# nurturenature/jepsen-tigerbeetle

Hardware: NVIDIA H100
Metric: configs explored/sec (time-to-verdict alongside) on 10k-op/32-client bank history (higher is better)
Workload: dtype int64

## Files before the change

### jepsen_tigerbeetle_b200/csrc/jtb_abi.cu

```cuda
#include <algorithm>
#include <chrono>
#include <cstdio>
#include <cstdlib>
#include <cstring>
#include <mutex>
#include <string>
#include <thread>
#include <type_traits>
#include <vector>

#include "jtb_wgl.cuh"
#include "jtb_level.cuh"
#include "jtb_scout.cuh"
#include "jtb_scans.cuh"
#include "jtb_table_bench.cuh"
#include "jtb_partition.cuh"
#include "jtb_monotonic.cuh"
#include "jtb_counter_bounds.cuh"
#include "jtb_transfer_lookups.cuh"
#include "jtb_read_explanations.cuh"
#include "jtb_read_gaps.cuh"
#include "jtb_transfer_placement.cuh"

using namespace jtb;
// ... 44 lines not shown
            return -1;                                                                       \
        }                                                                                    \
    } while (0)

int ensure(jtb_ctx* ctx, DevBuf& b, size_t bytes) {
    if (bytes <= b.cap) return 0;
    if (b.p) CK(cudaFree(b.p));
    b.p = nullptr;
    b.cap = 0;
    size_t want = std::max<size_t>(bytes, 256);
    CK(cudaMalloc(&b.p, want));
    b.cap = want;
    return 0;
}

template <typename T>
int upload(jtb_ctx* ctx, DevBuf& b, const std::vector<T>& v) {
    ctx->stats[12] += v.size() * sizeof(T);
    if (ensure(ctx, b, v.size() * sizeof(T) + 64)) return -1;
    if (!v.empty()) CK(cudaMemcpyAsync(b.p, v.data(), v.size() * sizeof(T), cudaMemcpyHostToDevice, ctx->stream));
    return 0;
}

template <typename F>
int dispatch_model_kw(jtb_ctx* ctx, int kind, int kw, F&& f) {
    using std::integral_constant;
    if (kind == JTB_MODEL_SET) return f(integral_constant<int, JTB_MODEL_SET>(), integral_constant<int, 2>());
    auto by_kw = [&](auto model) -> int {
        switch (kw) {
        case 2: return f(model, integral_constant<int, 2>());
        case 4: return f(model, integral_constant<int, 4>());
        case 8: return f(model, integral_constant<int, 8>());
        }
        ctx->err = "unsupported key width";
        return -1;
    };
    return kind == JTB_MODEL_BANK ? by_kw(integral_constant<int, JTB_MODEL_BANK>())
                                  : by_kw(integral_constant<int, JTB_MODEL_CAS_REGISTER>());
}

template <int MODEL, int KW>
int launch_wgl(jtb_ctx* ctx, const WglParams& p, int neg_ok, int grid, size_t smem) {
    auto k = p.eager_reads ? wgl_search_kernel<MODEL, KW, JTB_CTAS_EAGER, true> : wgl_search_kernel<MODEL, KW, JTB_CTAS_EXACT, false>;
    CK(cudaFuncSetAttribute(k, cudaFuncAttributeMaxDynamicSharedMemorySize, (int)smem));
    k<<<grid, WGL_THREADS, smem, ctx->stream>>>(p, neg_ok);
    CK(cudaGetLastError());
    return 0;
}

template <int MODEL, int KW>
int launch_level(jtb_ctx* ctx, const LvParams& p, int neg_ok, bool eager, int* grid_out) {
    constexpr int EW = KW + (MODEL == JTB_MODEL_BANK ? 4 : 0);
    const bool beam = p.beam_w != 0;
    const size_t smem = (beam ? sizeof(LvScratch<KW, EW, MODEL == JTB_MODEL_BANK, true>)
                              : sizeof(LvScratch<KW, EW, MODEL == JTB_MODEL_BANK, false>)) * LV_WARPS;
    const bool nk = !(MODEL == JTB_MODEL_BANK && !neg_ok);
    const void* k;
#define JTB_LVK(E, N, B) (const void*)level_search_kernel<MODEL, KW, E, (MODEL == JTB_MODEL_BANK ? N : true), B>
    if (beam) k = eager ? (nk ? JTB_LVK(true, true, true) : JTB_LVK(true, false, true)) : (nk ? JTB_LVK(false, true, true) : JTB_LVK(false, false, true));
    else k = eager ? (nk ? JTB_LVK(true, true, false) : JTB_LVK(true, false, false)) : (nk ? JTB_LVK(false, true, false) : JTB_LVK(false, false, false));
#undef JTB_LVK
    CK(cudaFuncSetAttribute(k, cudaFuncAttributeMaxDynamicSharedMemorySize, (int)smem));
    int per_sm = 0;
    CK(cudaOccupancyMaxActiveBlocksPerMultiprocessor(&per_sm, k, LV_THREADS, smem));
    if (per_sm < 1) { ctx->err = "level engine: the kernel does not fit on an SM"; return -1; }
    per_sm = std::min(per_sm, JTB_LV_CTAS);
    const int grid = ctx->opts.search_ctas ? std::min<int>((int)ctx->opts.search_ctas, ctx->n_sms * per_sm) : ctx->n_sms * per_sm;
    if (grid > 1024) { ctx->err = "level engine: more CTAs than barrier release words"; return -1; }
    *grid_out = grid;
    LvParams pp = p;
    void* args[] = {&pp};
    CK(cudaLaunchCooperativeKernel(k, dim3(grid), dim3(LV_THREADS), args, smem, ctx->stream));
    return 0;
}

int search_level(jtb_ctx* ctx, const jtb_model* m, const Prepared& P, int n_shards, const std::vector<int>& searchable,
                 const std::vector<uint64_t>& init_entries, Ctrl& hc, double& kernel_s, uint64_t& configs, uint64_t& probes,
                 uint32_t beam_w = 0) {
    const int KW = P.key_words;
    const bool bank = m->kind == JTB_MODEL_BANK;
    const int EW = KW + (bank ? 4 : 0);
    const bool eager = !(ctx->opts.flags & JTB_OPT_NO_EAGER_READS);
    size_t free_b = 0, total_b = 0;
    CK(cudaMemGetInfo(&free_b, &total_b));
    const size_t reserve = (size_t)4 << 30;
    const size_t avail = ctx->table.cap + ctx->lv_buf[0].cap + ctx->lv_buf[1].cap + (free_b > reserve ? free_b - reserve : 0);
    size_t table_bytes = ctx->opts.table_bytes ? ctx->opts.table_bytes
                         : (getenv("JTB_LV_TABLE_MB") ? (size_t)atoll(getenv("JTB_LV_TABLE_MB")) << 20 : (size_t)1 << 30);
    table_bytes = std::min(table_bytes, avail / 3);
    size_t buf_bytes = getenv("JTB_LV_BUF_MB") ? (size_t)atoll(getenv("JTB_LV_BUF_MB")) << 20 : (size_t)512 << 20;
    buf_bytes = std::max<size_t>(std::min(buf_bytes, avail / 3), init_entries.size() * 8 + 4096);
    auto slots_of = [&](size_t bytes) { uint64_t s = 1; while (s * 2 * KW * 8 <= bytes) s <<= 1; return s; };
    uint64_t table_slots = slots_of(std::max(table_bytes, ctx->table.cap));
    auto ensure_table = [&](uint64_t slots) -> int {
        const void* before = ctx->table.p;
        if (ensure(ctx, ctx->table, slots * KW * 8)) return -1;
        if (ctx->table.p != before) ctx->table_dirty = ~(size_t)0;
        return 0;
    };
    if (ensure_table(table_slots)) return -1;
    if (ensure(ctx, ctx->lv_buf[0], std::max(buf_bytes, ctx->lv_buf[0].cap)) || ensure(ctx, ctx->lv_buf[1], std::max(buf_bytes, ctx->lv_buf[1].cap)) ||
        ensure(ctx, ctx->lv_ctrl, sizeof(LvCtrl)))
        return -1;
    uint64_t buf_cap = std::min(ctx->lv_buf[0].cap, ctx->lv_buf[1].cap) / ((size_t)EW * 8);
    if (beam_w) {
        if (ensure(ctx, ctx->lv_aux[0], buf_cap * 4 + 64) || ensure(ctx, ctx->lv_aux[1], buf_cap * 4 + 64) ||
            ensure(ctx, ctx->lv_beam, sizeof(LvBeam)))
            return -1;
        std::vector<LvBeam> hb(1);
        std::memset(hb.data(), 0, sizeof(LvBeam));
        for (int k = 0; k < 3; ++k)
            for (int s = 0; s < LV_BEAM_SHARDS; ++s) { hb[0].min_crashed[k][s] = 0x7fffffff; hb[0].max_rank[k][s] = -1; }
        for (int s : searchable) { hb[0].min_crashed[0][s] = 0; hb[0].max_rank[0][s] = (int)P.rank_base[s]; }
        CK(cudaMemcpyAsync(ctx->lv_beam.p, hb.data(), sizeof(LvBeam), cudaMemcpyHostToDevice, ctx->stream));
        CK(cudaMemsetAsync(ctx->lv_aux[0].p, 0, init_entries.size() / EW * 4 + 64, ctx->stream));
        CK(cudaStreamSynchronize(ctx->stream));
    }
    CK(cudaMemsetAsync(ctx->table.p, 0, std::min(ctx->table_dirty, (size_t)table_slots * KW * 8), ctx->stream));
    ctx->table_dirty = 0;
    LvCtrl lc;
    std::memset(&lc, 0, sizeof lc);
    lc.n_undecided = (int)searchable.size();
    CK(cudaMemcpyAsync(ctx->lv_ctrl.p, &lc, sizeof lc, cudaMemcpyHostToDevice, ctx->stream));
    CK(cudaMemcpyAsync(ctx->lv_buf[0].p, init_entries.data(), init_entries.size() * 8, cudaMemcpyHostToDevice, ctx->stream));
    LvParams p{};
    p.rows = (const int32_t*)ctx->rows.p;
    p.classes = (const ClassRec*)ctx->classes.p;
    p.cls_inv_pos = (const int32_t*)ctx->cls_inv.p;
    p.ctrl = (LvCtrl*)ctx->lv_ctrl.p;
    p.shard_found = (int*)ctx->found.p;
    p.shard_max_rank = (int*)ctx->maxrank.p;
    p.row_words = P.row_words;
    p.sum_off = P.sum_off;
    p.n_shards = n_shards;
    p.max_configs = ctx->opts.max_configs;
    p.time_budget_ns = (unsigned long long)ctx->opts.time_budget_ms * 1000000ull;
    p.narrow_max = getenv("JTB_LV_NARROW") ? (uint32_t)atoi(getenv("JTB_LV_NARROW")) : (uint32_t)(LV_WARPS * 8);
    p.slots_per_config = getenv("JTB_LV_SPC") ? (uint32_t)std::max(2, atoi(getenv("JTB_LV_SPC"))) : 16u;
    p.min_slots = 1ull << 16;
    std::memset(&p.init, 0, sizeof p.init);
    p.init.n_in = searchable.size();
    p.init.epoch = 1;
    p.init.s_in = 0; p.init.s_out = 1; p.init.s_spare = 2;
    p.init.contig = 1;
    p.init.beam_thr = -1;
    p.init.beam_frac = 1024;
    p.beam_w = beam_w;
    p.aux[0] = (uint32_t*)ctx->lv_aux[0].p;
    p.aux[1] = (uint32_t*)ctx->lv_aux[1].p;
    p.beam = (LvBeam*)ctx->lv_beam.p;
    p.init.win = 0;
    CK(cudaEventRecord(ctx->ev0, ctx->stream));
    int attempts = 0, grid = 0;
    unsigned long long max_window = 0, max_width = 0, narrow_levels = 0, max_probe = 0;
    const double t_begin = now_s();
    for (;;) {
        ++attempts;
        p.table = (uint64_t*)ctx->table.p;
        p.table_slots = table_slots;
        p.min_slots = std::min<uint64_t>(p.min_slots, table_slots);
        p.buf[0] = (uint64_t*)ctx->lv_buf[0].p;
        p.buf[1] = (uint64_t*)ctx->lv_buf[1].p;
        p.buf_cap = buf_cap;
        p.seg_cap = buf_cap / LV_NSEG;
        p.init.zeroed = table_slots;
        p.init.win = lv_window(p, p.init.n_in, 0);
        if (ctx->opts.time_budget_ms) {
            const double left = ctx->opts.time_budget_ms * 1e-3 - (now_s() - t_begin);
            p.time_budget_ns = (unsigned long long)(std::max(left, 1e-3) * 1e9);
        }
        const int neg_ok = bank ? m->negative_balances_ok : 0;
        if (int rc = dispatch_model_kw(ctx, m->kind, KW, [&](auto M, auto K) { return launch_level<M(), K()>(ctx, p, neg_ok, eager, &grid); }))
            return rc;
        CK(cudaMemcpyAsync(&lc, ctx->lv_ctrl.p, sizeof lc, cudaMemcpyDeviceToHost, ctx->stream));
        CK(cudaStreamSynchronize(ctx->stream));
        if (lc.abort) { ctx->err = "level engine: a grid barrier timed out (internal error)"; return -1; }
#ifdef JTB_LV_PROF
        if (beam_w && getenv("JTB_BEAM_TRACE")) {
            for (int i = 0; i < 2048 && (i == 0 || lc.trace[i][1]); ++i)
                if (i < 40 || i % 25 == 0)
                    fprintf(stderr, "[beam W=%u] attempt %d level %d n_out %d thr %d frac %d min_c %d max_r %d\n", beam_w, i, lc.trace[i][0],
                            lc.trace[i][1], lc.trace[i][2], lc.trace[i][3], lc.trace[i][4], lc.trace[i][5]);
        }
        {
            const double wide = (double)std::max<unsigned long long>(lc.prof[9], 1), att = (double)std::max<unsigned long long>(lc.prof[8], 1);
            fprintf(stderr, "[lv prof] attempts %llu (wide %llu)  per attempt, cycles: phase1 %.0f phase2 %.0f flush %.0f | per wide level: "
                    "attempt %.0f barrier %.0f collect %.0f\n", lc.prof[8], lc.prof[9], lc.prof[0] / att, lc.prof[1] / att, lc.prof[2] / att,
                    lc.prof[3] / wide, lc.prof[4] / wide, lc.prof[5] / wide);
            unsigned long long bmin = ~0ull, bmax = 0, bsum = 0, wmin = ~0ull, wmax = 0, wsum = 0;
            for (int i = 0; i < grid; ++i) {
                bmin = std::min(bmin, lc.prof_cta[i][0]); bmax = std::max(bmax, lc.prof_cta[i][0]); bsum += lc.prof_cta[i][0];
                wmin = std::min(wmin, lc.prof_cta[i][1]); wmax = std::max(wmax, lc.prof_cta[i][1]); wsum += lc.prof_cta[i][1];
            }
            fprintf(stderr, "[lv prof] per CTA over the launch, Mcycles: busy min %.1f avg %.1f max %.1f | barrier wait min %.1f avg %.1f max %.1f\n",
                    bmin * 1e-6, bsum * 1e-6 / grid, bmax * 1e-6, wmin * 1e-6, wsum * 1e-6 / grid, wmax * 1e-6);
        }
#endif
        probes += lc.probes;
        max_window = std::max(max_window, lc.max_window);
        max_width = std::max(max_width, lc.max_width);
        max_probe = std::max(max_probe, lc.max_probe_len);
        narrow_levels += lc.narrow_levels;
        ctx->table_dirty = std::max(ctx->table_dirty, (size_t)std::max<uint64_t>(lc.max_window, p.min_slots) * KW * 8);
        if (!(lc.fin.stop == 2 && lc.fin.cause == JTB_CAUSE_TABLE_FULL)) break;
        if (beam_w) break;
        CK(cudaMemGetInfo(&free_b, &total_b));
        const size_t have = ctx->table.cap + ctx->lv_buf[0].cap + ctx->lv_buf[1].cap;
        const size_t room = have + (free_b > reserve ? free_b - reserve : 0);
        const size_t new_table = std::min<size_t>((size_t)table_slots * KW * 8 * 4, (size_t)64 << 30);
        const size_t new_buf = std::min(ctx->lv_buf[0].cap, ctx->lv_buf[1].cap) * 4;
        if (new_table + 2 * new_buf + ctx->lv_buf[lc.fin.in_idx].cap > room) break;
        const int ii = lc.fin.in_idx;
        if (ctx->lv_buf[ii ^ 1].p) { CK(cudaFree(ctx->lv_buf[ii ^ 1].p)); ctx->lv_buf[ii ^ 1] = DevBuf(); }
        if (ctx->table.p) { CK(cudaFree(ctx->table.p)); ctx->table = DevBuf(); }
        DevBuf grown;
        if (ensure(ctx, grown, new_buf)) return -1;
        if (lc.fin.contig) {
            CK(cudaMemcpyAsync(grown.p, ctx->lv_buf[ii].p, (size_t)lc.fin.n_in * EW * 8, cudaMemcpyDeviceToDevice, ctx->stream));
        } else {
            size_t off = 0;
            const size_t seg_cap = buf_cap / LV_NSEG;
            for (int sg = 0; sg < LV_NSEG; ++sg) {
                const size_t n = (size_t)lc.seg[lc.fin.s_in][sg].n;
                if (!n) continue;
                CK(cudaMemcpyAsync((char*)grown.p + off * EW * 8, (const char*)ctx->lv_buf[ii].p + (size_t)sg * seg_cap * EW * 8,
                                   n * EW * 8, cudaMemcpyDeviceToDevice, ctx->stream));
                off += n;
            }
            if (off != lc.fin.n_in) { ctx->err = "level engine: segment counts do not add up"; return -1; }
        }
        CK(cudaStreamSynchronize(ctx->stream));
        CK(cudaFree(ctx->lv_buf[ii].p));
        ctx->lv_buf[ii] = grown;
        if (ensure(ctx, ctx->lv_buf[ii ^ 1], new_buf)) return -1;
        table_slots = slots_of(new_table);
        if (ensure_table(table_slots)) return -1;
        CK(cudaMemsetAsync(ctx->table.p, 0, (size_t)table_slots * KW * 8, ctx->stream));
        ctx->table_dirty = 0;
        buf_cap = new_buf / ((size_t)EW * 8);
        LvState r = lc.fin;
        r.stop = 0; r.cause = 0; r.boost = 0; r.attempt = 0; r.epoch = 1;
        r.s_in = 0; r.s_out = 1; r.s_spare = 2; r.contig = 1;
        p.init = r;
        const int undecided = lc.n_undecided;
        std::memset(&lc, 0, sizeof lc);
        lc.n_undecided = undecided;
        CK(cudaMemcpyAsync(ctx->lv_ctrl.p, &lc, sizeof lc, cudaMemcpyHostToDevice, ctx->stream));
    }
    CK(cudaEventRecord(ctx->ev1, ctx->stream));
    CK(cudaStreamSynchronize(ctx->stream));
    float ms = 0;
    CK(cudaEventElapsedTime(&ms, ctx->ev0, ctx->ev1));
    kernel_s = ms * 1e-3;
    configs = lc.fin.total;
    std::memset(&hc, 0, sizeof hc);
    hc.stop = lc.fin.stop;
    hc.cause = lc.fin.cause;
    hc.configs = lc.fin.total;
    hc.probes = probes;
    hc.n_undecided = lc.n_undecided;
    unsigned long long* st = ctx->stats;
    st[0] = configs; st[1] = probes; st[2] = lc.fin.level + 1; st[3] = max_width; st[4] = narrow_levels; st[5] = 0;
    st[6] = max_probe; st[7] = max_window; st[8] = (unsigned long long)grid; st[9] = buf_cap;
    st[10] = (unsigned long long)attempts; st[11] = (unsigned long long)(ms * 1e3);
    st[12] += init_entries.size() * 8 + sizeof(LvCtrl) + (size_t)n_shards * 4;
    st[13] = (unsigned long long)attempts * sizeof(LvCtrl) + (size_t)n_shards * 8;
    st[14] = (unsigned long long)attempts;
    st[19] = 1;
    return 0;
}

struct ScoutGuard {
    jtb_ctx* ctx;
    bool active = false;
    explicit ScoutGuard(jtb_ctx* c) : ctx(c) {}
    int stop() {
        if (!active) return 0;
        active = false;
        static const unsigned long long one = 1;
        cudaError_t e = cudaMemcpyAsync((unsigned long long*)ctx->sc_ctl.p + 1, &one, 8, cudaMemcpyHostToDevice, ctx->stream);
        if (e == cudaSuccess) e = cudaStreamSynchronize(ctx->scout_stream);
        if (e != cudaSuccess) { ctx->err = std::string("stopping the scouts: ") + cudaGetErrorString(e); return -1; }
        return 0;
    }
    ~ScoutGuard() { stop(); }
};

template <typename K>
int preload(jtb_ctx* ctx, K kernel) {
    cudaFuncAttributes a;
    CK(cudaFuncGetAttributes(&a, kernel));
    return 0;
}

template <int MODEL, int KW>
// ... 800 lines not shown
```

### jepsen_tigerbeetle_b200/csrc/jtb_expand.h

```cpp
#pragma once
#include <cstdint>

#include "jtb_prep.h"

#if defined(__CUDACC__)
#define JTB_HD __host__ __device__ __forceinline__
#else
#define JTB_HD inline
#endif

namespace jtb {

constexpr uint64_t XKEY_VALID = 1ull << 63;
constexpr uint32_t XRANK_MASK = 0x1fffffffu;

struct I4 {
    int32_t x, y, z, w;
};

JTB_HD I4 ld_i4(const int32_t* p) {
#if defined(__CUDA_ARCH__)
    const int4 v = __ldg(reinterpret_cast<const int4*>(p));
    return I4{v.x, v.y, v.z, v.w};
#else
// ... 187 lines not shown
        }
#pragma unroll
        for (int i = 0; i < KW; ++i) ch.w[i] = w[i];
        int cgj = gj;
        if (t == rslot) advance(T, ch.w[1], cgj);
        else ch.w[1] |= 1ull << t;
        ch.w[0] = XKEY_VALID | ((uint64_t)(uint32_t)cgj << 32) | (REG ? (uint64_t)(uint32_t)creg : 0ull);
        ch.cgj = cgj;
        ch.done = cgj >= gj_end;
        return true;
    }

    JTB_HD void load_transfer(int t, Child<KW>& ch) const {
        const I4 op = ld_i4(row + ROW_EXTRA + t * SW);
        ch.amt = op.y; ch.d = op.z; ch.c = op.w;
    }

    JTB_HD bool child_class(const ExpandTables& T, int ci, bool neg_ok, Child<KW>& ch) const {
        const int32_t* q = reinterpret_cast<const int32_t*>(T.classes + cls_base + ci);
        const I4 b = ld_i4(q + 4);
        const int shift = b.w & 0xff, width = b.w >> 8;
        uint64_t field = 0;
#pragma unroll
        for (int i = 1; i < KW; ++i) if (i == b.z) field = w[i];
        const int count = (int)((field >> shift) & ((1ull << width) - 1));
        if (count >= b.y) return false;
        if (ld_i32(T.cls_inv_pos + b.x + count) >= fr_pos) return false;
        const I4 op = ld_i4(q);
        if (op.x & OP_IMPOSSIBLE) return false;
        int32_t creg = reg;
        ch.amt = 0; ch.d = 0; ch.c = 0;
        if constexpr (REG) {
            const int f = op.x & 0xff;
            if (f == JTB_F_WRITE) creg = op.y;
            else if (f == JTB_F_CAS) { if (reg != op.y) return false; creg = op.z; }
            else if (!(op.y == JTB_NIL || op.y == reg)) return false;
        } else if constexpr (BANK) {
            if ((op.x & 0xff) != JTB_F_TRANSFER) return false;
            ch.amt = op.y; ch.d = op.z; ch.c = op.w;
            if (!neg_ok && balance_of(op.z) - op.y < 0) return false;
        } else {
            if ((op.x & 0xff) != JTB_F_ADD) return false;
        }
#pragma unroll
        for (int i = 0; i < KW; ++i) ch.w[i] = w[i];
#pragma unroll
        for (int i = 1; i < KW; ++i) if (i == b.z) ch.w[i] += 1ull << shift;
        ch.w[0] = XKEY_VALID | ((uint64_t)(uint32_t)gj << 32) | (REG ? (uint64_t)(uint32_t)creg : 0ull);
        ch.cgj = gj;
        ch.done = false;
        return true;
    }

    JTB_HD bool next(const ExpandTables& T, bool neg_ok, Child<KW>& ch) {
        while (todo) {
            const int t = ctz64(todo);
            todo &= todo - 1;
            if (child_slot(T, t, neg_ok, ch)) return true;
        }
        while (cls_i < ncls) {
            const int ci = cls_i++;
            if (child_class(T, ci, neg_ok, ch)) return true;
        }
        return false;
    }
};

}
```

### jepsen_tigerbeetle_b200/csrc/jtb_level.cuh

```cuda
#pragma once
#include "jtb_expand.h"
#include "jtb_wgl.cuh"

namespace jtb {

#ifndef JTB_LV_WARPS
#define JTB_LV_WARPS 8
#endif
#ifndef JTB_LV_CTAS
#define JTB_LV_CTAS 3
#endif
constexpr int LV_WARPS = JTB_LV_WARPS;
constexpr int LV_THREADS = LV_WARPS * 32;
constexpr int LV_STAGE = 64;
constexpr int LV_MAX_PROBE = 128;
constexpr int LV_CLS_WORDS = 8;
constexpr uint64_t LV_TAG_MASK = 0x3full << 56;
constexpr int64_t LV_MAX_RANKS = 1ll << 24;

constexpr int LV_NSEG = 64;
constexpr unsigned LV_F_DECIDED = 1, LV_F_GIVEUP = 2, LV_F_RETRY = 4;

struct LvSeg {
    alignas(128) unsigned long long n;
};
constexpr int LV_BEAM_BINS = 1024;
constexpr int LV_BEAM_SHARDS = 16;
struct LvBeam {
    unsigned hist[3][LV_BEAM_BINS];
    int min_crashed[3][LV_BEAM_SHARDS];
    int max_rank[3][LV_BEAM_SHARDS];
};
__host__ __device__ inline int lv_beam_key(int crashed, int min_crashed, int rank, int max_rank) {
    int c = crashed - min_crashed, r = max_rank + 2 - rank;
    c = c < 0 ? 0 : (c > 15 ? 15 : c);
    r = r < 0 ? 0 : (r > 63 ? 63 : r);
    return c * 64 + r;
}

struct LvState {
    unsigned long long level, attempt, n_in, total;
    int epoch, in_idx, boost, stop, cause;
    int s_in, s_out, s_spare;
    int contig;
    unsigned long long win;
    int beam_thr, beam_frac;
    unsigned long long zeroed;
};
struct LvRelease {
    alignas(32) unsigned long long gen;
};
struct LvCtrl {
    alignas(128) LvSeg seg[3][LV_NSEG];
    alignas(128) unsigned flags[3][32];
    alignas(128) LvState pub;
    alignas(128) int n_undecided;
    int abort;
    alignas(128) unsigned long long probes;
    unsigned long long max_probe_len, max_width, max_window, narrow_levels, retries, t0, t1;
    LvState fin;
    unsigned long long prof[16];
    unsigned long long prof_cta[1024][2];
    int trace[2048][6];
    alignas(128) LvRelease arrive[1024];
    alignas(128) LvRelease release[1024];
};

struct LvParams {
    const int32_t* rows;
    const ClassRec* classes;
    const int32_t* cls_inv_pos;
    uint64_t* table;
    uint64_t table_slots;
    uint64_t* buf[2];
    uint32_t* aux[2];
    LvBeam* beam;
    uint32_t beam_w;
    uint64_t buf_cap;
    uint64_t seg_cap;
    LvCtrl* ctrl;
    int* shard_found;
    int* shard_max_rank;
    int row_words, sum_off, n_shards;
    unsigned long long max_configs;
    unsigned long long time_budget_ns;
    LvState init;
    uint32_t narrow_max;
    uint32_t slots_per_config;
    uint64_t min_slots;
};

template <int KW, int EW, bool BAL, bool BEAM>
struct LvScratch {
    uint64_t w[32][KW];
    uint64_t todo[32], rd_ok[32];
    uint64_t cls_todo[32][BEAM ? LV_CLS_WORDS : 1];
    int32_t bal[BAL ? 32 : 1][8];
    int32_t hdr[32][6];
    uint32_t start[36];
    uint32_t crashed[BEAM ? 32 : 1];
    uint32_t stage_aux[BEAM ? LV_STAGE : 1];
    uint64_t stage[LV_STAGE][EW];
};

__device__ __forceinline__ int select64(uint64_t m, int k) {
    const uint32_t lo = (uint32_t)m;
    const int c = __popc(lo);
    return k < c ? (int)__fns(lo, 0, k + 1) : 32 + (int)__fns((uint32_t)(m >> 32), 0, k - c + 1);
}

__device__ __forceinline__ void lv_load_state(LvState& dst, const LvState* src) {
    static_assert(sizeof(LvState) % 8 == 0, "LvState is copied as 64-bit words");
    uint64_t* d = reinterpret_cast<uint64_t*>(&dst);
    const uint64_t* q = reinterpret_cast<const uint64_t*>(src);
#pragma unroll
    for (int i = 0; i < (int)(sizeof(LvState) / 8); ++i) d[i] = ldcg64(q + i);
}

template <int KW>
__device__ __forceinline__ int lv_insert(uint64_t* table, uint64_t mask, const uint64_t (&k)[KW], uint64_t tag, int* plen) {
    uint64_t idx = hash_key<KW>(k) & mask;
    const uint64_t mine0 = k[0] | tag;
    for (int i = 0; i < LV_MAX_PROBE; ++i) {
        uint64_t* slot = table + idx * KW;
        K128 cur = ldcg128(slot);
        for (int round = 0; round < 2; ++round) {
            const bool free_slot = !(cur.lo >> 63) || (cur.lo & LV_TAG_MASK) != tag;
            if (!free_slot) break;
            const K128 mine{KW == 2 ? mine0 : (mine0 | KEY_LOCK), k[1]};
            const K128 old = cas128(slot, cur, mine);
            if (old.lo == cur.lo && old.hi == cur.hi) {
                if constexpr (KW > 2) {
#pragma unroll
                    for (int x = 2; x < KW; ++x) slot[x] = k[x];
                    __threadfence();
                    *(volatile uint64_t*)slot = mine0;
                }
                *plen = i + 1;
                return 1;
            }
            cur = old;
        }
        if constexpr (KW == 2) {
            if ((cur.lo & ~LV_TAG_MASK) == k[0] && cur.hi == k[1]) { *plen = i + 1; return 0; }
        } else {
            if ((cur.lo & ~(LV_TAG_MASK | KEY_LOCK)) == k[0] && cur.hi == k[1]) {
                while (cur.lo & KEY_LOCK) cur.lo = ldcg64(slot);
                __threadfence();
                bool same = true;
#pragma unroll
                for (int x = 2; x < KW; ++x) same &= ldcg64(slot + x) == k[x];
                if (same) { *plen = i + 1; return 0; }
            }
        }
        idx = (idx + 1) & mask;
    }
    *plen = LV_MAX_PROBE;
    return -1;
}

#ifdef JTB_LV_PROF
#define LV_PROF(i, t0) do { if (blockIdx.x == 0 && threadIdx.x == 0) { const long long t_ = clock64(); ctrl->prof[i] += t_ - (t0); (t0) = t_; } } while (0)
#else
#define LV_PROF(i, t0) do { } while (0)
#endif

__device__ __forceinline__ bool lv_grid_barrier(LvCtrl* ctrl, unsigned long long& gen, bool patient) {
    __shared__ int s_ok;
    gen++;
    if (threadIdx.x == 0) s_ok = 1;
    __syncthreads();
#ifdef JTB_LV_PROF
    __shared__ long long s_t_leave;
    long long t_arrive = 0;
    if (threadIdx.x == 0) {
        t_arrive = clock64();
        if (gen > 1) ctrl->prof_cta[blockIdx.x][0] += t_arrive - s_t_leave;
    }
#endif
    const unsigned long long limit = patient ? 900000000000ull : 20000000000ull;
    auto wait_for = [&](const unsigned long long* word) {
        unsigned ns = 20, spins = 0;
        unsigned long long t_wait = 0;
        while (ld_volatile(word) < gen) {
            if (patient) { __nanosleep(ns); if (ns < 400) ns += ns; }
            if ((++spins & 0xfff) == 0) {
                const unsigned long long now = globaltimer();
                if (!t_wait) t_wait = now;
                if (now - t_wait > limit || ld_volatile(&ctrl->abort)) { atomicExch(&ctrl->abort, 1); s_ok = 0; return; }
            }
        }
    };
    if (blockIdx.x == 0) {
        __threadfence();
        for (unsigned i = threadIdx.x + 1; i < gridDim.x; i += blockDim.x) wait_for(&ctrl->arrive[i].gen);
        __syncthreads();
        __threadfence();
        for (unsigned i = threadIdx.x + 1; i < gridDim.x; i += blockDim.x) *(volatile unsigned long long*)&ctrl->release[i].gen = gen;
    } else if (threadIdx.x == 0) {
        __threadfence();
        *(volatile unsigned long long*)&ctrl->arrive[blockIdx.x].gen = gen;
        wait_for(&ctrl->release[blockIdx.x].gen);
        __threadfence();
    }
#ifdef JTB_LV_PROF
    if (threadIdx.x == 0) {
        s_t_leave = clock64();
        ctrl->prof_cta[blockIdx.x][1] += s_t_leave - t_arrive;
    }
#endif
    __syncthreads();
    return s_ok != 0;
}

__host__ __device__ inline uint64_t lv_pow2ceil(uint64_t x) {
#if defined(__CUDA_ARCH__)
    return x <= 1 ? 1ull : 1ull << (64 - __clzll((long long)(x - 1)));
#else
    uint64_t s = 1;
    while (s < x) s <<= 1;
    return s;
#endif
}

__host__ __device__ inline uint64_t lv_window(const LvParams& p, unsigned long long n_in, int boost) {
    uint64_t want = (uint64_t)n_in * p.slots_per_config;
    if (want < p.min_slots) want = p.min_slots;
    uint64_t s = lv_pow2ceil(want);
    for (int b = 0; b < boost && s < p.table_slots; ++b) s <<= 2;
    return s < p.table_slots ? s : p.table_slots;
}

__device__ __forceinline__ void lv_advance(const LvParams& p, LvState& st, unsigned long long cnt, bool over, unsigned flags) {
    st.attempt++;
    st.epoch = (st.epoch + 1) & 63;
    const int o_in = st.s_in, o_out = st.s_out, o_spare = st.s_spare;
    if (flags & LV_F_GIVEUP) { st.stop = 2; st.cause = (int)(flags >> 8); return; }
    if (flags & LV_F_RETRY) {
        if (st.win >= p.table_slots) { st.stop = 2; st.cause = JTB_CAUSE_TABLE_FULL; return; }
        st.boost++;
        st.win = lv_window(p, st.n_in, st.boost);
        st.s_out = o_spare; st.s_spare = o_out;
        return;
    }
    if (over) { st.stop = 2; st.cause = JTB_CAUSE_TABLE_FULL; return; }
    st.total += cnt;
    if (flags & LV_F_DECIDED) { st.stop = 1; return; }
    if (cnt == 0) { st.stop = 1; return; }
    if (p.max_configs && st.total >= p.max_configs) { st.stop = 2; st.cause = JTB_CAUSE_BUDGET; return; }
    st.level++;
    st.n_in = cnt;
    st.in_idx ^= 1;
    st.contig = 0;
    st.beam_thr = -1;
    st.win = lv_window(p, st.n_in, st.boost);
    st.s_in = o_out; st.s_out = o_spare; st.s_spare = o_in;
}

template <int MODEL, int KW, bool EAGER, bool NEGOK, bool BEAM>
__global__ void __launch_bounds__(LV_THREADS, JTB_LV_CTAS) level_search_kernel(const LvParams p) {
    constexpr bool neg_ok = NEGOK;
    constexpr int CLS_WORDS = BEAM ? LV_CLS_WORDS : 1;
    using L = EntryLayout<MODEL, KW>;
    constexpr int EW = L::EW;
    constexpr bool BAL = L::HAS_BAL;
    constexpr unsigned FULL = 0xffffffffu;
    using Scratch = LvScratch<KW, EW, BAL, BEAM>;
    extern __shared__ __align__(16) unsigned char lv_smem[];
    __shared__ LvState s_state;
    __shared__ unsigned long long s_seg_start[LV_NSEG + 1];
    const int tid = threadIdx.x, lane = tid & 31, warp = tid >> 5;
    const unsigned lt_mask = (1u << lane) - 1;
    Scratch& S = reinterpret_cast<Scratch*>(lv_smem)[warp];
    LvCtrl* ctrl = p.ctrl;
    ExpandTables T;
    T.rows = p.rows; T.classes = p.classes; T.cls_inv_pos = p.cls_inv_pos; T.row_words = p.row_words; T.sum_off = p.sum_off;

    LvState st = p.init;
    unsigned long long bar_gen = 0;
    unsigned long long my_probes = 0;
    int my_max_probe = 0;
    int wit_shard = -1, wit_rank = -1;
    if (blockIdx.x == 0 && tid == 0) ctrl->t0 = globaltimer();
    if (tid <= LV_NSEG) s_seg_start[tid] = tid == 0 ? 0 : st.n_in;
    __syncthreads();

    auto entry_of = [&](const LvState& a, unsigned long long idx, unsigned long long& eidx) -> const uint64_t* {
        int lo = 0, hi = LV_NSEG;
        while (hi - lo > 1) {
            const int mid = (lo + hi) >> 1;
            if (s_seg_start[mid] <= idx) lo = mid; else hi = mid;
        }
        eidx = (unsigned long long)lo * p.seg_cap + (idx - s_seg_start[lo]);
        return p.buf[a.in_idx] + eidx * EW;
    };

    auto run_attempt = [&](const LvState& a, unsigned first_chunk, unsigned chunk_stride) {
        unsigned G = 32, g_log = 5;
        if (a.n_in < 32ull * chunk_stride) {
            const unsigned q = ((unsigned)a.n_in + chunk_stride - 1) / chunk_stride;
            g_log = q <= 1 ? 0 : 32 - __clz(q - 1);
            G = 1u << g_log;
        }
        const unsigned n_chunks = (unsigned)((a.n_in + G - 1) >> g_log);
        if (first_chunk >= n_chunks) return;
        uint64_t* out = p.buf[a.in_idx ^ 1];
        unsigned* res_flags = &ctrl->flags[a.s_out][0];
        const unsigned my_seg = first_chunk % LV_NSEG;
        unsigned long long* my_cnt = &ctrl->seg[a.s_out][my_seg].n;
        uint64_t* my_out = out + (unsigned long long)my_seg * p.seg_cap * EW;
        const uint64_t wmask = a.win - 1;
        const uint64_t tag = (uint64_t)a.epoch << 56;
        unsigned stg_head = 0, stg_tail = 0;
        int bt_shard = -1, bt_min = 0x7fffffff, bt_max = -1;
        auto flush = [&](unsigned n) {
            unsigned long long base = 0;
            if (lane == 0) base = atomicAdd(my_cnt, (unsigned long long)n);
            base = __shfl_sync(FULL, base, 0);
            if (base + n <= p.seg_cap) {
                uint64_t* dst = my_out + base * EW;
                for (unsigned x = lane; x < n * EW; x += 32) {
                    const unsigned e = x / EW, k = x - e * EW;
                    dst[x] = S.stage[(stg_head + e) % LV_STAGE][k];
                }
                if (BEAM && (unsigned)lane < n)
                    p.aux[a.in_idx ^ 1][(unsigned long long)my_seg * p.seg_cap + base + lane] = S.stage_aux[(stg_head + lane) % LV_STAGE];
            }
            stg_head += n;
            __syncwarp();
        };
#ifdef JTB_LV_PROF
        long long tp = clock64();
        if (blockIdx.x == 0 && threadIdx.x == 0) ctrl->prof[8]++;
#endif
        for (unsigned chunk = first_chunk; chunk < n_chunks; chunk += chunk_stride) {
            const unsigned long long idx = (unsigned long long)chunk * G + lane;
            const bool have = (unsigned)lane < G && idx < a.n_in;
            uint64_t todo = 0;
            unsigned n_cls_children = 0;
            {
                Expander<MODEL, KW, EAGER> X;
                X.todo = 0; X.rd_ok = 0; X.ncls = 0; X.cls_i = 0;
                X.fr_pos = 0; X.shard = 0; X.gj_end = 0; X.cls_base = 0; X.rslot = 0;
                if (have) {
                    unsigned long long eidx;
                    const uint64_t* e = entry_of(a, idx, eidx);
                    unsigned crashed = 0;
                    if constexpr (BEAM) crashed = __ldcg(p.aux[a.in_idx] + eidx);
#pragma unroll
                    for (int i = 0; i < KW; ++i) X.w[i] = ldcg64(e + i);
                    if constexpr (BAL) {
#pragma unroll
                        for (int i = 0; i < 4; ++i) {
                            const uint64_t v = ldcg64(e + KW + i);
                            X.bal[2 * i] = (int32_t)(uint32_t)v;
                            X.bal[2 * i + 1] = (int32_t)(uint32_t)(v >> 32);
                        }
                    }
                    const int shard = X.load_header(T);
                    bool alive = !(p.n_shards > 1 && ld_volatile(&p.shard_found[shard]));
                    if constexpr (BEAM) {
                        S.crashed[lane] = crashed & 0xffffu;
                        if (a.beam_thr >= 0) {
                            const int key = (int)(crashed >> 16);
                            alive = alive && (key < a.beam_thr ||
                                              (key == a.beam_thr && (int)((hash_key<KW>(X.w) >> 17) & 1023) < a.beam_frac));
                        }
                    }
                    X.begin(T, alive);
                    todo = X.todo;
#pragma unroll
                    for (int cw = 0; cw < CLS_WORDS; ++cw) S.cls_todo[lane][cw] = 0;
                    if (X.cls_i == 0) {
                        uint64_t cw_bits = 0;
                        for (int ci = 0; ci < X.ncls; ++ci) {
                            const int32_t* q = reinterpret_cast<const int32_t*>(T.classes + X.cls_base + ci);
                            const I4 b = ld_i4(q + 4);
                            const int shift = b.w & 0xff, width = b.w >> 8;
                            uint64_t field = 0;
#pragma unroll
                            for (int i = 1; i < KW; ++i) if (i == b.z) field = X.w[i];
                            const int count = (int)((field >> shift) & ((1ull << width) - 1));
                            if (count < b.y && ld_i32(T.cls_inv_pos + b.x + count) < X.fr_pos) { cw_bits |= 1ull << (ci & 63); ++n_cls_children; }
                            if ((ci & 63) == 63 || ci == X.ncls - 1) { S.cls_todo[lane][ci >> 6] = cw_bits; cw_bits = 0; }
                        }
                    }
#pragma unroll
                    for (int i = 0; i < KW; ++i) S.w[lane][i] = X.w[i];
                    if constexpr (BAL) {
#pragma unroll
                        for (int i = 0; i < 8; ++i) S.bal[lane][i] = X.bal[i];
                    }
                    S.rd_ok[lane] = X.rd_ok;
                    S.hdr[lane][0] = X.fr_pos; S.hdr[lane][1] = X.shard; S.hdr[lane][2] = X.gj_end;
                    S.hdr[lane][3] = X.cls_base; S.hdr[lane][4] = X.rslot; S.hdr[lane][5] = X.ncls;
                }
                S.todo[lane] = todo;
            }
            unsigned c = (unsigned)__popcll(todo) + n_cls_children;
            unsigned incl = c;
#pragma unroll
            for (int o = 1; o < 32; o <<= 1) {
                const unsigned v = __shfl_up_sync(FULL, incl, o);
                if (lane >= o) incl += v;
            }
            LV_PROF(0, tp);
            S.start[lane] = incl - c;
            const unsigned total = __shfl_sync(FULL, incl, 31);
            if (lane == 0) S.start[32] = total;
            __syncwarp();
            for (unsigned g0 = 0; g0 < total; g0 += 32) {
                const unsigned g = g0 + lane;
                const bool act = g < total;
                Child<KW> ch;
                bool is_new = false;
                int owner = 0;
                unsigned child_crashed = 0;
                if (act) {
                    int lo = 0, hi = 32;
                    while (hi - lo > 1) {
                        const int mid = (lo + hi) >> 1;
                        if (S.start[mid] <= g) lo = mid; else hi = mid;
                    }
                    owner = lo;
                    const int k = (int)(g - S.start[owner]);
                    Expander<MODEL, KW, EAGER> Y;
#pragma unroll
                    for (int i = 0; i < KW; ++i) Y.w[i] = S.w[owner][i];
                    if constexpr (BAL && !NEGOK) {
#pragma unroll
                        for (int i = 0; i < 8; ++i) Y.bal[i] = S.bal[owner][i];
                    }
                    Y.rd_ok = S.rd_ok[owner];
                    Y.gj = (int)((Y.w[0] >> 32) & XRANK_MASK);
                    Y.reg = (int32_t)(uint32_t)Y.w[0];
                    Y.row = T.rows + (size_t)Y.gj * T.row_words;
                    Y.fr_pos = S.hdr[owner][0]; Y.shard = S.hdr[owner][1]; Y.gj_end = S.hdr[owner][2];
                    Y.cls_base = S.hdr[owner][3]; Y.rslot = S.hdr[owner][4]; Y.ncls = S.hdr[owner][5];
                    const uint64_t otodo = S.todo[owner];
                    const int ns = __popcll(otodo);
                    bool ok;
                    int t_slot = 0;
                    if constexpr (BEAM) child_crashed = S.crashed[owner] + (k >= ns ? 1u : 0u);
                    if (k < ns) { t_slot = select64(otodo, k); ok = Y.child_slot(T, t_slot, neg_ok, ch, true); }
                    else {
                        int kk = k - ns, cw = 0;
                        for (; cw < CLS_WORDS - 1; ++cw) {
                            const int pc = __popcll(S.cls_todo[owner][cw]);
                            if (kk < pc) break;
                            kk -= pc;
                        }
                        ok = Y.child_class(T, cw * 64 + select64(S.cls_todo[owner][cw], kk), neg_ok, ch);
                    }
                    if (ok) {
                        if (ch.done) {
                            if (atomicExch(&p.shard_found[Y.shard], 1) == 0) {
                                if (atomicSub(&ctrl->n_undecided, 1) == 1) atomicOr(res_flags, LV_F_DECIDED);
                            }
                        } else {
                            int plen;
                            const int r = lv_insert<KW>(p.table, wmask, ch.w, tag, &plen);
                            my_probes++;
                            my_max_probe = max(my_max_probe, plen);
                            if (r < 0) atomicOr(res_flags, LV_F_RETRY);
                            is_new = r == 1;
                            if constexpr (BAL) {
                                if (is_new && ch.d < 0) Y.load_transfer(t_slot, ch);
                            }
                            if (is_new && ch.cgj > Y.gj && (wit_shard != Y.shard || wit_rank < ch.cgj)) {
                                wit_shard = Y.shard; wit_rank = ch.cgj;
                                atomicMax(&p.shard_max_rank[Y.shard], ch.cgj);
                            }
                            if (BEAM && is_new) {
                                LvBeam* bm = p.beam;
                                const int key = lv_beam_key((int)child_crashed, __ldcg(&bm->min_crashed[a.s_in][Y.shard]), ch.cgj,
                                                            __ldcg(&bm->max_rank[a.s_in][Y.shard]));
                                atomicAdd(&bm->hist[a.s_out][key], 1u);
                                child_crashed = min(child_crashed, 0xffffu) | ((unsigned)key << 16);
                                if (bt_shard != Y.shard) { bt_shard = Y.shard; bt_min = 0x7fffffff; bt_max = -1; }
                                const int cc = (int)(child_crashed & 0xffffu);
                                if (cc < bt_min) { bt_min = cc; atomicMin(&bm->min_crashed[a.s_out][Y.shard], bt_min); }
                                if (ch.cgj > bt_max) { bt_max = ch.cgj; atomicMax(&bm->max_rank[a.s_out][Y.shard], bt_max); }
                            }
                        }
                    }
                }
                const unsigned newm = __ballot_sync(FULL, is_new);
                if (newm) {
                    if (is_new) {
                        uint64_t* e = S.stage[(stg_tail + __popc(newm & lt_mask)) % LV_STAGE];
                        if constexpr (BEAM) S.stage_aux[(stg_tail + __popc(newm & lt_mask)) % LV_STAGE] = child_crashed;
#pragma unroll
                        for (int i = 0; i < KW; ++i) e[i] = ch.w[i];
                        if constexpr (BAL) {
                            int32_t b[8];
#pragma unroll
                            for (int i = 0; i < 8; ++i) b[i] = S.bal[owner][i];
                            if (ch.amt) {
#pragma unroll
                                for (int i = 0; i < 8; ++i) {
                                    if (i == ch.d) b[i] -= ch.amt;
                                    if (i == ch.c) b[i] += ch.amt;
                                }
                            }
#pragma unroll
                            for (int i = 0; i < 4; ++i) e[KW + i] = u64_of(b[2 * i], b[2 * i + 1]);
                        }
                    }
                    stg_tail += __popc(newm);
                    __syncwarp();
                    if (stg_tail - stg_head >= 32) flush(32);
                }
            }
            __syncwarp();
// ... 27 lines not shown
                if (t0 + t1 > cap) {
                    unsigned mine = 0;
                    const unsigned* hh = p.beam->hist[a.s_out];
#pragma unroll 8
                    for (int i = 0; i < 32; ++i) mine += *(volatile const unsigned*)&hh[lane * 32 + i];
                    unsigned incl_h = mine;
#pragma unroll
                    for (int o = 1; o < 32; o <<= 1) {
                        const unsigned v = __shfl_up_sync(FULL, incl_h, o);
                        if (lane >= o) incl_h += v;
                    }
                    const unsigned reach = __ballot_sync(FULL, incl_h >= cap);
                    if (reach) {
                        const int wl = __ffs(reach) - 1;
                        if (lane == wl) {
                            unsigned long long run = incl_h - mine;
                            int b = 0;
                            unsigned in_bin = 1;
                            for (; b < 32; ++b) {
                                in_bin = *(volatile const unsigned*)&hh[lane * 32 + b];
                                if (run + in_bin >= cap) break;
                                run += in_bin;
                            }
                            thr = lane * 32 + min(b, 31);
                            frac = (int)min(1024ull, (cap - min(cap, run)) * 1024ull / max(in_bin, 1u) + 1ull);
                        }
                        thr = __shfl_sync(FULL, thr, wl);
                        frac = __shfl_sync(FULL, frac, wl);
                    }
                }
            }
            if (lane == 0 && !nx.stop && !((fl & LV_F_RETRY))) { nx.beam_thr = thr; nx.beam_frac = frac; }
#ifdef JTB_LV_PROF
            if (BEAM && blockIdx.x == 0 && lane == 0 && a.attempt < 2048) {
                int* tr = ctrl->trace[a.attempt];
                tr[0] = (int)a.level; tr[1] = (int)(t0 + t1); tr[2] = thr; tr[3] = frac;
                tr[4] = *(volatile int*)&p.beam->min_crashed[a.s_out][0]; tr[5] = *(volatile int*)&p.beam->max_rank[a.s_out][0];
            }
#endif
            const bool repeated = (__shfl_sync(FULL, fl, 0) & LV_F_RETRY) != 0;
            if (!repeated) {
                s_seg_start[lane + 1] = i0;
                s_seg_start[lane + 33] = t0 + i1;
                if (lane == 0) s_seg_start[0] = 0;
            }
            if (lane == 0) s_state = nx;
        }
        __syncthreads();
        a = s_state;
    };

    auto zero_fill = [&](uint64_t from, uint64_t to) {
        ulonglong2* t = reinterpret_cast<ulonglong2*>(p.table);
        const uint64_t n16 = (to - from) * KW / 2, off = from * KW / 2;
        for (uint64_t i = (uint64_t)blockIdx.x * LV_THREADS + tid; i < n16; i += (uint64_t)gridDim.x * LV_THREADS)
            t[off + i] = make_ulonglong2(0, 0);
    };
    auto reset_spare = [&](const LvState& a) {
        ctrl->seg[a.s_spare][lane].n = 0;
        ctrl->seg[a.s_spare][lane + 32].n = 0;
        if (lane == 0) ctrl->flags[a.s_spare][0] = 0;
        if constexpr (BEAM) {
            for (int i = lane; i < LV_BEAM_BINS; i += 32) p.beam->hist[a.s_spare][i] = 0;
            if (lane < LV_BEAM_SHARDS) { p.beam->min_crashed[a.s_spare][lane] = 0x7fffffff; p.beam->max_rank[a.s_spare][lane] = -1; }
        }
    };

    for (;;) {
        if (st.stop) break;
        const bool narrow = st.n_in <= p.narrow_max;
        {
            const uint64_t win = st.win;
            if (win > st.zeroed) {
                zero_fill(st.zeroed, win);
                st.zeroed = win;
                if (!lv_grid_barrier(ctrl, bar_gen, false)) break;
            }
        }
        if (!narrow) {
            if (blockIdx.x == 0 && warp == LV_WARPS - 1) {
                reset_spare(st);
                if (lane == 0) {
                    if (p.time_budget_ns && globaltimer() - ctrl->t0 > p.time_budget_ns)
                        atomicOr(&ctrl->flags[st.s_out][0], LV_F_GIVEUP | ((unsigned)JTB_CAUSE_BUDGET << 8));
                    if (st.n_in > ctrl->max_width) ctrl->max_width = st.n_in;
                    if (st.win > ctrl->max_window) ctrl->max_window = st.win;
                }
            }
#ifdef JTB_LV_PROF
            long long tw = clock64();
#endif
            run_attempt(st, (unsigned)warp * gridDim.x + blockIdx.x, (unsigned)gridDim.x * LV_WARPS);
            LV_PROF(3, tw);
            if (!lv_grid_barrier(ctrl, bar_gen, false)) break;
            LV_PROF(4, tw);
            collect(st);
            LV_PROF(5, tw);
#ifdef JTB_LV_PROF
            if (blockIdx.x == 0 && threadIdx.x == 0) ctrl->prof[9]++;
#endif
            if (!st.stop && st.n_in <= p.narrow_max && !lv_grid_barrier(ctrl, bar_gen, false)) break;
        } else {
            if (blockIdx.x == 0) {
                for (;;) {
                    if (warp == LV_WARPS - 1) {
                        reset_spare(st);
                        if (lane == 0) {
// ... 51 lines not shown
```

Baseline: 3.494 billion.

## Add sleep-set partial-order reduction to bank level search

Adds sleep sets to the level-synchronous search for the bank model when negative balances are allowed and eager reads and beam are off. Each hash table slot now carries a 128-bit sleep mask stamped per attempt, and the table is double-banked by level parity, so a node can look up its parent-level sleep mask. Commuting transitions already explored from a sibling are then removed from its todo set. This aims to cut redundant interleavings of independent operations. In exchange table slots grow considerably, each insert adds a 128-bit CAS merge, and slots_per_config drops to 4 to compensate for memory.

New measurement: 3.882 billion (median of 6 runs). 11.1% higher.

```diff
diff --git a/jepsen_tigerbeetle_b200/csrc/jtb_abi.cu b/jepsen_tigerbeetle_b200/csrc/jtb_abi.cu
--- a/jepsen_tigerbeetle_b200/csrc/jtb_abi.cu
+++ b/jepsen_tigerbeetle_b200/csrc/jtb_abi.cu
@@ -120,9 +120,11 @@
 int launch_level(jtb_ctx* ctx, const LvParams& p, int neg_ok, bool eager, int* grid_out) {
     constexpr int EW = KW + (MODEL == JTB_MODEL_BANK ? 4 : 0);
     const bool beam = p.beam_w != 0;
-    const size_t smem = (beam ? sizeof(LvScratch<KW, EW, MODEL == JTB_MODEL_BANK, true>)
-                              : sizeof(LvScratch<KW, EW, MODEL == JTB_MODEL_BANK, false>)) * LV_WARPS;
     const bool nk = !(MODEL == JTB_MODEL_BANK && !neg_ok);
+    const bool sleep = MODEL == JTB_MODEL_BANK && nk && !eager && !beam;
+    const size_t smem = (beam ? sizeof(LvScratch<KW, EW, MODEL == JTB_MODEL_BANK, true, false>)
+                              : sleep ? sizeof(LvScratch<KW, EW, MODEL == JTB_MODEL_BANK, false, true>)
+                                      : sizeof(LvScratch<KW, EW, MODEL == JTB_MODEL_BANK, false, false>)) * LV_WARPS;
     const void* k;
 #define JTB_LVK(E, N, B) (const void*)level_search_kernel<MODEL, KW, E, (MODEL == JTB_MODEL_BANK ? N : true), B>
     if (beam) k = eager ? (nk ? JTB_LVK(true, true, true) : JTB_LVK(true, false, true)) : (nk ? JTB_LVK(false, true, true) : JTB_LVK(false, false, true));
@@ -149,6 +151,8 @@
     const bool bank = m->kind == JTB_MODEL_BANK;
     const int EW = KW + (bank ? 4 : 0);
     const bool eager = !(ctx->opts.flags & JTB_OPT_NO_EAGER_READS);
+    const bool sleep = bank && m->negative_balances_ok && !eager && !beam_w;
+    const size_t slot_bytes = (size_t)(sleep ? 2 * (KW + 2) : KW) * 8;
     size_t free_b = 0, total_b = 0;
     CK(cudaMemGetInfo(&free_b, &total_b));
     const size_t reserve = (size_t)4 << 30;
@@ -158,11 +162,11 @@
     table_bytes = std::min(table_bytes, avail / 3);
     size_t buf_bytes = getenv("JTB_LV_BUF_MB") ? (size_t)atoll(getenv("JTB_LV_BUF_MB")) << 20 : (size_t)512 << 20;
     buf_bytes = std::max<size_t>(std::min(buf_bytes, avail / 3), init_entries.size() * 8 + 4096);
-    auto slots_of = [&](size_t bytes) { uint64_t s = 1; while (s * 2 * KW * 8 <= bytes) s <<= 1; return s; };
+    auto slots_of = [&](size_t bytes) { uint64_t s = 1; while (s * 2 * slot_bytes <= bytes) s <<= 1; return s; };
     uint64_t table_slots = slots_of(std::max(table_bytes, ctx->table.cap));
     auto ensure_table = [&](uint64_t slots) -> int {
         const void* before = ctx->table.p;
-        if (ensure(ctx, ctx->table, slots * KW * 8)) return -1;
+        if (ensure(ctx, ctx->table, slots * slot_bytes)) return -1;
         if (ctx->table.p != before) ctx->table_dirty = ~(size_t)0;
         return 0;
     };
@@ -184,7 +188,7 @@
         CK(cudaMemsetAsync(ctx->lv_aux[0].p, 0, init_entries.size() / EW * 4 + 64, ctx->stream));
         CK(cudaStreamSynchronize(ctx->stream));
     }
-    CK(cudaMemsetAsync(ctx->table.p, 0, std::min(ctx->table_dirty, (size_t)table_slots * KW * 8), ctx->stream));
+    CK(cudaMemsetAsync(ctx->table.p, 0, std::min(ctx->table_dirty, (size_t)table_slots * slot_bytes), ctx->stream));
     ctx->table_dirty = 0;
     LvCtrl lc;
     std::memset(&lc, 0, sizeof lc);
@@ -204,7 +208,7 @@
     p.max_configs = ctx->opts.max_configs;
     p.time_budget_ns = (unsigned long long)ctx->opts.time_budget_ms * 1000000ull;
     p.narrow_max = getenv("JTB_LV_NARROW") ? (uint32_t)atoi(getenv("JTB_LV_NARROW")) : (uint32_t)(LV_WARPS * 8);
-    p.slots_per_config = getenv("JTB_LV_SPC") ? (uint32_t)std::max(2, atoi(getenv("JTB_LV_SPC"))) : 16u;
+    p.slots_per_config = getenv("JTB_LV_SPC") ? (uint32_t)std::max(2, atoi(getenv("JTB_LV_SPC"))) : (sleep ? 4u : 16u);
     p.min_slots = 1ull << 16;
     std::memset(&p.init, 0, sizeof p.init);
     p.init.n_in = searchable.size();
@@ -269,13 +273,13 @@
         max_width = std::max(max_width, lc.max_width);
         max_probe = std::max(max_probe, lc.max_probe_len);
         narrow_levels += lc.narrow_levels;
-        ctx->table_dirty = std::max(ctx->table_dirty, (size_t)std::max<uint64_t>(lc.max_window, p.min_slots) * KW * 8);
+        ctx->table_dirty = std::max(ctx->table_dirty, (size_t)std::max<uint64_t>(lc.max_window, p.min_slots) * slot_bytes);
         if (!(lc.fin.stop == 2 && lc.fin.cause == JTB_CAUSE_TABLE_FULL)) break;
         if (beam_w) break;
         CK(cudaMemGetInfo(&free_b, &total_b));
         const size_t have = ctx->table.cap + ctx->lv_buf[0].cap + ctx->lv_buf[1].cap;
         const size_t room = have + (free_b > reserve ? free_b - reserve : 0);
-        const size_t new_table = std::min<size_t>((size_t)table_slots * KW * 8 * 4, (size_t)64 << 30);
+        const size_t new_table = std::min<size_t>((size_t)table_slots * slot_bytes * 4, (size_t)64 << 30);
         const size_t new_buf = std::min(ctx->lv_buf[0].cap, ctx->lv_buf[1].cap) * 4;
         if (new_table + 2 * new_buf + ctx->lv_buf[lc.fin.in_idx].cap > room) break;
         const int ii = lc.fin.in_idx;
@@ -303,12 +307,13 @@
         if (ensure(ctx, ctx->lv_buf[ii ^ 1], new_buf)) return -1;
         table_slots = slots_of(new_table);
         if (ensure_table(table_slots)) return -1;
-        CK(cudaMemsetAsync(ctx->table.p, 0, (size_t)table_slots * KW * 8, ctx->stream));
+        CK(cudaMemsetAsync(ctx->table.p, 0, (size_t)table_slots * slot_bytes, ctx->stream));
         ctx->table_dirty = 0;
         buf_cap = new_buf / ((size_t)EW * 8);
         LvState r = lc.fin;
         r.stop = 0; r.cause = 0; r.boost = 0; r.attempt = 0; r.epoch = 1;
         r.s_in = 0; r.s_out = 1; r.s_spare = 2; r.contig = 1;
+        r.zwin = 0;
         p.init = r;
         const int undecided = lc.n_undecided;
         std::memset(&lc, 0, sizeof lc);
diff --git a/jepsen_tigerbeetle_b200/csrc/jtb_expand.h b/jepsen_tigerbeetle_b200/csrc/jtb_expand.h
--- a/jepsen_tigerbeetle_b200/csrc/jtb_expand.h
+++ b/jepsen_tigerbeetle_b200/csrc/jtb_expand.h
@@ -263,6 +263,16 @@
         return true;
     }
 
+    JTB_HD uint64_t sleep(uint64_t z) {
+        z &= todo;
+        todo &= ~z;
+        return z;
+    }
+    JTB_HD static uint64_t sleep_proposal(uint64_t z, uint64_t fired, uint64_t rd_ok, int t) {
+        const uint64_t same = ((rd_ok >> t) & 1ull) ? rd_ok : ~rd_ok;
+        return (z | (fired & ((1ull << t) - 1))) & same;
+    }
+
     JTB_HD bool next(const ExpandTables& T, bool neg_ok, Child<KW>& ch) {
         while (todo) {
             const int t = ctz64(todo);
diff --git a/jepsen_tigerbeetle_b200/csrc/jtb_level.cuh b/jepsen_tigerbeetle_b200/csrc/jtb_level.cuh
--- a/jepsen_tigerbeetle_b200/csrc/jtb_level.cuh
+++ b/jepsen_tigerbeetle_b200/csrc/jtb_level.cuh
@@ -46,6 +46,8 @@
     unsigned long long win;
     int beam_thr, beam_frac;
     unsigned long long zeroed;
+    unsigned long long zwin, zstamp;
+    int zepoch, zpad;
 };
 struct LvRelease {
     alignas(32) unsigned long long gen;
@@ -90,10 +92,11 @@
     uint64_t min_slots;
 };
 
-template <int KW, int EW, bool BAL, bool BEAM>
+template <int KW, int EW, bool BAL, bool BEAM, bool SLEEP>
 struct LvScratch {
     uint64_t w[32][KW];
     uint64_t todo[32], rd_ok[32];
+    uint64_t zz[SLEEP ? 32 : 1];
     uint64_t cls_todo[32][BEAM ? LV_CLS_WORDS : 1];
     int32_t bal[BAL ? 32 : 1][8];
     int32_t hdr[32][6];
@@ -117,12 +120,25 @@
     for (int i = 0; i < (int)(sizeof(LvState) / 8); ++i) d[i] = ldcg64(q + i);
 }
 
-template <int KW>
-__device__ __forceinline__ int lv_insert(uint64_t* table, uint64_t mask, const uint64_t (&k)[KW], uint64_t tag, int* plen) {
+__device__ __forceinline__ void lv_sleep_merge(uint64_t* zslot, uint64_t prop, uint64_t stamp) {
+    K128 cur = ldcg128(zslot);
+    for (;;) {
+        const bool mine = cur.hi == stamp;
+        const uint64_t z = mine ? (cur.lo & prop) : prop;
+        if (mine && z == cur.lo) return;
+        const K128 old = cas128(zslot, cur, K128{z, stamp});
+        if (old.lo == cur.lo && old.hi == cur.hi) return;
+        cur = old;
+    }
+}
+
+template <int KW, int SW, bool SLEEP>
+__device__ __forceinline__ int lv_insert(uint64_t* table, uint64_t mask, const uint64_t (&k)[KW], uint64_t tag, int* plen,
+                                         uint64_t prop = 0, uint64_t stamp = 0) {
     uint64_t idx = hash_key<KW>(k) & mask;
     const uint64_t mine0 = k[0] | tag;
     for (int i = 0; i < LV_MAX_PROBE; ++i) {
-        uint64_t* slot = table + idx * KW;
+        uint64_t* slot = table + idx * SW;
         K128 cur = ldcg128(slot);
         for (int round = 0; round < 2; ++round) {
             const bool free_slot = !(cur.lo >> 63) || (cur.lo & LV_TAG_MASK) != tag;
@@ -136,13 +152,18 @@
                     __threadfence();
                     *(volatile uint64_t*)slot = mine0;
                 }
+                if constexpr (SLEEP) lv_sleep_merge(slot + KW, prop, stamp);
                 *plen = i + 1;
                 return 1;
             }
             cur = old;
         }
         if constexpr (KW == 2) {
-            if ((cur.lo & ~LV_TAG_MASK) == k[0] && cur.hi == k[1]) { *plen = i + 1; return 0; }
+            if ((cur.lo & ~LV_TAG_MASK) == k[0] && cur.hi == k[1]) {
+                if constexpr (SLEEP) lv_sleep_merge(slot + KW, prop, stamp);
+                *plen = i + 1;
+                return 0;
+            }
         } else {
             if ((cur.lo & ~(LV_TAG_MASK | KEY_LOCK)) == k[0] && cur.hi == k[1]) {
                 while (cur.lo & KEY_LOCK) cur.lo = ldcg64(slot);
@@ -150,13 +171,35 @@
                 bool same = true;
 #pragma unroll
                 for (int x = 2; x < KW; ++x) same &= ldcg64(slot + x) == k[x];
-                if (same) { *plen = i + 1; return 0; }
+                if (same) {
+                    if constexpr (SLEEP) lv_sleep_merge(slot + KW, prop, stamp);
+                    *plen = i + 1;
+                    return 0;
+                }
             }
         }
         idx = (idx + 1) & mask;
     }
     *plen = LV_MAX_PROBE;
     return -1;
+}
+
+template <int KW, int SW>
+__device__ __forceinline__ uint64_t lv_sleep_mask(const uint64_t* table, uint64_t mask, const uint64_t (&k)[KW], uint64_t tag,
+                                                  uint64_t stamp) {
+    uint64_t idx = hash_key<KW>(k) & mask;
+    for (int i = 0; i < LV_MAX_PROBE; ++i) {
+        const K128 cur = ldcg128(table + idx * SW), zcur = ldcg128(table + idx * SW + KW);
+        if (!(cur.lo >> 63) || (cur.lo & LV_TAG_MASK) != tag) return 0;
+        if ((cur.lo & ~(LV_TAG_MASK | KEY_LOCK)) == k[0] && cur.hi == k[1]) {
+            bool same = true;
+#pragma unroll
+            for (int x = 2; x < KW; ++x) same &= ldcg64(table + idx * SW + x) == k[x];
+            if (same) return zcur.hi == stamp ? zcur.lo : 0ull;
+        }
+        idx = (idx + 1) & mask;
+    }
+    return 0;
 }
 
 #ifdef JTB_LV_PROF
@@ -232,6 +275,8 @@
 }
 
 __device__ __forceinline__ void lv_advance(const LvParams& p, LvState& st, unsigned long long cnt, bool over, unsigned flags) {
+    const unsigned long long done_win = st.win, done_stamp = st.attempt + 1;
+    const int done_epoch = st.epoch;
     st.attempt++;
     st.epoch = (st.epoch + 1) & 63;
     const int o_in = st.s_in, o_out = st.s_out, o_spare = st.s_spare;
@@ -255,6 +300,7 @@
     st.beam_thr = -1;
     st.win = lv_window(p, st.n_in, st.boost);
     st.s_in = o_out; st.s_out = o_spare; st.s_spare = o_in;
+    st.zwin = done_win; st.zstamp = done_stamp; st.zepoch = done_epoch;
 }
 
 template <int MODEL, int KW, bool EAGER, bool NEGOK, bool BEAM>
@@ -265,7 +311,10 @@
     constexpr int EW = L::EW;
     constexpr bool BAL = L::HAS_BAL;
     constexpr unsigned FULL = 0xffffffffu;
-    using Scratch = LvScratch<KW, EW, BAL, BEAM>;
+    constexpr bool SLEEP = MODEL == JTB_MODEL_BANK && NEGOK && !EAGER && !BEAM;
+    constexpr int TW = KW + (SLEEP ? 2 : 0);
+    constexpr int SW = SLEEP ? 2 * TW : KW;
+    using Scratch = LvScratch<KW, EW, BAL, BEAM, SLEEP>;
     extern __shared__ __align__(16) unsigned char lv_smem[];
     __shared__ LvState s_state;
     __shared__ unsigned long long s_seg_start[LV_NSEG + 1];
@@ -368,6 +417,12 @@
                         }
                     }
                     X.begin(T, alive);
+                    if constexpr (SLEEP) {
+                        const uint64_t z = a.zwin ? lv_sleep_mask<KW, SW>(p.table + ((a.level & 1) ^ 1) * TW, a.zwin - 1, X.w,
+                                                                         (uint64_t)a.zepoch << 56, a.zstamp)
+                                                  : 0ull;
+                        S.zz[lane] = X.sleep(z);
+                    }
                     todo = X.todo;
 #pragma unroll
                     for (int cw = 0; cw < CLS_WORDS; ++cw) S.cls_todo[lane][cw] = 0;
@@ -440,7 +495,7 @@
                     const uint64_t otodo = S.todo[owner];
                     const int ns = __popcll(otodo);
                     bool ok;
-                    int t_slot = 0;
+                    int t_slot = -1;
                     if constexpr (BEAM) child_crashed = S.crashed[owner] + (k >= ns ? 1u : 0u);
                     if (k < ns) { t_slot = select64(otodo, k); ok = Y.child_slot(T, t_slot, neg_ok, ch, true); }
                     else {
@@ -459,7 +514,9 @@
                             }
                         } else {
                             int plen;
-                            const int r = lv_insert<KW>(p.table, wmask, ch.w, tag, &plen);
+                            const uint64_t prop = SLEEP && t_slot >= 0 ? Y.sleep_proposal(S.zz[owner], otodo, Y.rd_ok, t_slot) : 0ull;
+                            const int r = lv_insert<KW, SW, SLEEP>(p.table + (SLEEP ? (a.level & 1) * TW : 0), wmask, ch.w, tag,
+                                                                   &plen, prop, a.attempt + 1);
                             my_probes++;
                             my_max_probe = max(my_max_probe, plen);
                             if (r < 0) atomicOr(res_flags, LV_F_RETRY);
@@ -593,7 +650,7 @@
 
     auto zero_fill = [&](uint64_t from, uint64_t to) {
         ulonglong2* t = reinterpret_cast<ulonglong2*>(p.table);
-        const uint64_t n16 = (to - from) * KW / 2, off = from * KW / 2;
+        const uint64_t n16 = (to - from) * SW / 2, off = from * SW / 2;
         for (uint64_t i = (uint64_t)blockIdx.x * LV_THREADS + tid; i < n16; i += (uint64_t)gridDim.x * LV_THREADS)
             t[off + i] = make_ulonglong2(0, 0);
     };
```
